# t-0hmura/pdb2reaction

Hardware: AMD Instinct MI355X
Metric: path_opt_string_iterations_per_s (higher is better)
Workload: dtype bf16x3-split

## Files before the change

### pdb2reaction_amd/csrc/umx_api.hip

```cpp
#include "umx_engine.h"
#include "umx_launch.h"
#include "umx_workspace.h"
#include "umx_periodic.h"
#include "umx_virial.h"
#include "umx_plan.h"
#include "umx_weights.h"
#include "umx_experts.h"

#define NOT_MERGED "expert-form weights are loaded but not merged: call umx_set_expert_coefficients first (then umx_set_system)"

namespace {
int energy_forces_dev_impl(umx_engine* eng, int n_images, const PosPtr d_pos, double* d_energy, float* d_forces, double* d_virial, void* hip_stream) {
  if (!eng) return UMX_ERR_ARG;
  if (eng->need_merge()) return fail(eng, UMX_ERR_ARG, "umx_energy_forces: " NOT_MERGED);
  if (!eng->have_system) return fail(eng, UMX_ERR_ARG, "umx_energy_forces: bind a system first (umx_set_system)");
  if (n_images <= 0 || !(d_pos.f || d_pos.d) || !d_energy) return fail(eng, UMX_ERR_ARG, "umx_energy_forces: bad arguments");
  if (d_virial && !d_forces) return fail(eng, UMX_ERR_ARG, "umx_energy_forces_virial: the virial comes out of the reverse pass: ask for the forces too");
  if (eng->gp_plan) return fail(eng, UMX_ERR_ARG, "umx_energy_forces: a graph-parallel evaluation is in progress (finish it with umx_gp_step)");
  CHK(periodic_check_images(eng, n_images, "umx_energy_forces"));
  HIPCHK(eng, hipSetDevice(eng->dev));
  return energy_forces_on(eng, static_cast<hipStream_t>(hip_stream), n_images, d_pos, d_energy, d_forces, d_virial);
}

template <typename P>
// ... 145 lines not shown
  if (hipGetDeviceCount(&n) != hipSuccess || n <= 0) { g_create_err = "umx_create: no HIP device visible"; return UMX_ERR_NO_DEVICE; }
  if (device_ordinal < 0 || device_ordinal >= n) { g_create_err = "umx_create: device ordinal out of range"; return UMX_ERR_ARG; }
  hipDeviceProp_t prop;
  if (hipGetDeviceProperties(&prop, device_ordinal) != hipSuccess) { g_create_err = "umx_create: hipGetDeviceProperties failed"; return UMX_ERR_HIP; }
  if (std::string(prop.gcnArchName).rfind("gfx950", 0) != 0) {
    g_create_err = std::string("umx_create: device is ") + prop.gcnArchName + ", this library is built for gfx950 only";
    return UMX_ERR_NO_DEVICE;
  }
  umx_engine* e = new umx_engine();
  e->dev = device_ordinal;
  if (const char* ev = std::getenv("UMX_STREAMS")) e->n_lanes = std::atoi(ev) >= 2 ? 2 : (std::atoi(ev) == 1 ? 1 : 0);
  if (const char* ev = std::getenv("UMX_LANES_AUTO_EDGES")) e->lanes_auto_edges = std::max(0L, std::atol(ev));
  if (const char* ev = std::getenv("UMX_FORCE_PARTS")) e->force_parts = std::max(0, std::min(16, std::atoi(ev)));
  if (const char* ev = std::getenv("UMX_RECOMPUTE")) e->recompute = std::max(0, std::min(2, std::atoi(ev)));
  if (const char* ev = std::getenv("UMX_WS_GB")) e->ws_cap_default = (size_t)std::max(0L, std::atol(ev)) << 30;
  if (const char* ev = std::getenv("UMX_WS_EAGER")) e->ws_eager = std::atoi(ev) != 0;
  if (const char* ev = std::getenv("UMX_WS_SOFT_EDGES")) e->ws_soft_edges = std::max(1L, std::atol(ev));
  if (const char* ev = std::getenv("UMX_NODE_F64")) e->node_f64_on = std::atoi(ev) != 0;
  if (const char* ev = std::getenv("UMX_GRID_F64")) e->grid_f64 = std::atoi(ev) != 0;
  if (const char* ev = std::getenv("UMX_ALT_ROWS")) e->odd_sign = std::atoi(ev) != 0 ? -1.0f : 1.0f;
  if (const char* ev = std::getenv("UMX_LOW_SEP")) e->low_sep = std::atoi(ev);
  if (const char* ev = std::getenv("UMX_GEMM_HALF")) e->gemm_half = std::atoi(ev);
  if (const char* ev = std::getenv("UMX_ALIGN_PLANES")) e->align = std::atoi(ev);
  int prio_lo = 0, prio_hi = 0;
  if (hipSetDevice(device_ordinal) != hipSuccess || hipDeviceGetStreamPriorityRange(&prio_lo, &prio_hi) != hipSuccess ||
      hipStreamCreateWithFlags(&e->stream, hipStreamNonBlocking) != hipSuccess ||
      hipStreamCreateWithPriority(&e->stream2, hipStreamNonBlocking, prio_hi) != hipSuccess ||
      hipEventCreateWithFlags(&e->ev_fork, hipEventDisableTiming) != hipSuccess || hipEventCreateWithFlags(&e->ev_join, hipEventDisableTiming) != hipSuccess ||
      hipEventCreateWithFlags(&e->ev_tok[0], hipEventDisableTiming) != hipSuccess || hipEventCreateWithFlags(&e->ev_tok[1], hipEventDisableTiming) != hipSuccess ||
      hipEventCreateWithFlags(&e->ev_done, hipEventDisableTiming) != hipSuccess || hipMalloc(&e->d_flags, 4 * sizeof(int)) != hipSuccess ||
      hipMemset(e->d_flags, 0, 4 * sizeof(int)) != hipSuccess) {
    g_create_err = "umx_create: hipSetDevice/hipStreamCreate failed";
    delete e;
    return UMX_ERR_HIP;
  }
  *out = e;
  return UMX_OK;
}


int umx_destroy(umx_engine* eng) {
  if (!eng) return UMX_OK;
  gp_clear(eng);
  (void)hipSetDevice(eng->dev);
  (void)hipStreamSynchronize(eng->stream);
  for (auto& r : eng->prof) { (void)hipEventDestroy(r.a); (void)hipEventDestroy(r.b); }
// ... 156 lines not shown
    return fail(eng, UMX_ERR_ARG, "umx_gp_begin: recompute mode 2 (umx_set_recompute / UMX_RECOMPUTE=2) is a one-GPU plan; the multi-GPU graph-parallel mode "
                                  "keeps every rank's activations stored: set mode 0 or 1 on the engines that take part");
  if (eng->pin_on)
    return fail(eng, UMX_ERR_ARG, "umx_gp_begin: a graph is pinned (umx_pin_graph) and the graph-parallel entries build their own: call umx_unpin_graph first");
  if (eng->pbc_on && eng->n_cells > 1)
    return fail(eng, UMX_ERR_ARG, "umx_gp_begin: one image, but umx_set_cells bound cells for " + std::to_string(eng->n_cells) +
                                  " images: the graph-parallel mode takes per-image cells only when exactly one is bound");
  if (eng->gp_plan) gp_clear(eng);
  HIPCHK(eng, hipSetDevice(eng->dev));
  eng->gp = true; eng->gp_lo = node_lo; eng->gp_hi = node_hi;
  const int st = energy_forces_on(eng, static_cast<hipStream_t>(hip_stream), 1, d_pos, d_energy, d_forces, d_virial);
  if (st != UMX_OK) gp_clear(eng);
  return st;
}

int umx_gp_step(umx_engine* eng, float** d_buf, size_t* count, int* done) {
  if (!eng || !d_buf || !count || !done) return UMX_ERR_ARG;
  if (!eng->gp_plan) return fail(eng, UMX_ERR_ARG, "umx_gp_step: no graph-parallel evaluation in progress (umx_gp_begin)");
  HIPCHK(eng, hipSetDevice(eng->dev));
  hipStream_t own = eng->stream;
  eng->stream = eng->gp_stream;
  *d_buf = nullptr; *count = 0; *done = 0;
  const Seg* stop = nullptr;
  int st = eng->gp_plan->run_to_sync(eng->gp_at, &stop);
  eng->stream = own;
  if (stop) { *d_buf = stop->sync_buf; *count = stop->sync_count; return UMX_OK; }
  if (st == UMX_OK) {
    *done = 1;
    eng->ran_on_caller = true;
    hipError_t e = hipEventRecord(eng->ev_done, eng->gp_stream);
    if (e != hipSuccess) st = fail(eng, UMX_ERR_HIP, std::string("umx_gp_step: ") + hipGetErrorName(e));
  }
  gp_clear(eng);
  return st;
}

namespace {
struct PeerState {
  hipEvent_t ev_in[PEER_MAX] = {}, ev_out[PEER_MAX] = {};
  int ev_dev[PEER_MAX];
  std::set<std::pair<int, int>> enabled;
  PeerState() { for (int& d : ev_dev) d = -1; }
} g_peer;

int peer_fail(int code, const std::string& msg) { g_create_err = msg; return code; }

#define PEERCHK(expr)                                                                                          \
// ... 273 lines not shown
```

### pdb2reaction_amd/csrc/umx_engine.h

```cpp
#pragma once
#include <hip/hip_runtime.h>
#include <algorithm>
#include <cmath>
#include <cstdio>
#include <cstdlib>
#include <chrono>
#include <cstring>
#include <functional>
#include <initializer_list>
#include <map>
#include <memory>
#include <set>
#include <string>
#include <type_traits>
#include <vector>

#include "../../include/umx.h"
#include "umx_common.h"
#include "umx_gemm.h"
#include "umx_gemm_pl.h"
#include "umx_gemm_q.h"
#include "umx_kernels_pl.h"
#include "umx_kernels.h"
#include "umx_radial.h"
// ... 86 lines not shown
struct WS {
  int *deg, *row_ptr, *stats;
  float* xs[2 * NL + 1];
  float* xn[NL];
  float *xn2, *ffhg, *xf, *pre1, *pre2, *enode;
  float* gspre[NL];
  float* ffh[NL];
  float* ffg1[NL];
  float* ffg2[NL];
  float *gridA, *gridB;
  float *G0, *G1, *G2, *ggs, *n128a, *n128b;
  int *esrc, *edst, *ez, *out_ptr, *out_cur, *out_edge;
  float *evec, *frame, *dedd, *dedd_rad, *tau, *tau2, *gvec;
  float* h1pre[NL + 1];
  float* h2pre[NL + 1];
  float *ra, *rad_deg;
  float* rad[NL];
  float* hg[NL];
  float* msg[NL];
  float *xrot, *hid, *gmsg, *ghg, *gy1, *grad, *e128a;
  unsigned short *y1pl, *hidpl, *a2pl, *gmsgpl, *ghgpl, *gradpl;
};

struct Seg { bool matrix; std::function<int()> fn; float* sync_buf = nullptr; size_t sync_count = 0; };
struct Plan {
  std::vector<Seg> segs;
  void stream(std::function<int()> f) { segs.push_back({false, std::move(f)}); }
  void matrix(std::function<int()> f) { segs.push_back({true, std::move(f)}); }
  void sync(float* buf, size_t count) { Seg sg{false, nullptr}; sg.sync_buf = buf; sg.sync_count = count; segs.push_back(std::move(sg)); }
  int run_to_sync(size_t& at, const Seg** stop) {
    *stop = nullptr;
    while (at < segs.size()) {
      Seg& sg = segs[at++];
      if (sg.sync_buf) { *stop = &sg; return UMX_OK; }
      const int st = sg.fn();
      if (st != UMX_OK) return st;
    }
    return UMX_OK;
  }
};

}

struct umx_engine {
  int dev = 0;
  hipStream_t stream = nullptr;
  hipEvent_t ev_done = nullptr;
  bool ran_on_caller = false;
  int* d_flags = nullptr;
  hipStream_t stream2 = nullptr;
  hipEvent_t ev_fork = nullptr, ev_join = nullptr;
  hipEvent_t ev_tok[2] = {nullptr, nullptr};
  Precision prec;
  std::string precision;
  int low_sep = 3;
  int gemm_half = 5;
  int align = 2;
  float odd_sign = -1.0f;
  bool node_ctx = false;
  bool node_f64_on = true;
  int n_lanes = 0;
  long lanes_auto_edges = 0;
  int stream_cap = 512;
  bool throttle = false;
  bool gp = false; long gp_lo = 0, gp_hi = 0;
  std::unique_ptr<Plan> gp_plan;
  std::unique_ptr<WS> gp_ws;
  size_t gp_at = 0;
  hipStream_t gp_stream = nullptr;
  std::string err;
  bool have_weights = false;
  float* d_w = nullptr;
  float* d_dw = nullptr;
  double* d_dtab = nullptr;
  unsigned short* d_bw = nullptr;
  std::map<const float*, PlaneCopy> planes;
  std::map<std::string, Tensor> wt;
  std::vector<float> h_w;
  size_t n_w = 0, n_dw = 0, n_bw = 0;
  int n_experts = 0;
  bool experts_merged = false;
  float* d_ex = nullptr;
  MergeJob* d_mjobs = nullptr; PackJob* d_pjobs = nullptr; unsigned* d_mx = nullptr;
  int n_mjobs = 0, n_pjobs = 0, merge_blocks = 0, pack_blocks = 0;
  std::vector<const float*> f16_keys;
// ... 82 lines not shown
  std::vector<ProfRec> prof;
  size_t prof_used = 0;
  bool dbg_on = false;
  std::map<std::string, std::vector<char>> dbg;
};

namespace {

#define HIPCHK(eng, expr)                                                                         \
  do {                                                                                            \
    hipError_t _e = (expr);                                                                       \
    if (_e != hipSuccess) {                                                                       \
      (eng)->err = std::string(#expr) + ": " + hipGetErrorName(_e) + " (" + hipGetErrorString(_e) + ")"; \
      return UMX_ERR_HIP;                                                                         \
    }                                                                                             \
  } while (0)

#define CHK(expr) do { int _s = (expr); if (_s != UMX_OK) return _s; } while (0)

int fail(umx_engine* e, int code, const std::string& msg) { e->err = msg; return code; }

inline unsigned nblk(long n, int per) { return (unsigned)((n + per - 1) / per); }

struct DevBuf {
  void** p; size_t bytes;
  template <class T> DevBuf(T*& ptr, size_t count) : p(reinterpret_cast<void**>(&ptr)), bytes(count * sizeof(T)) {}
};
template <class Cap>
int grow(umx_engine* eng, Cap& cap, Cap new_cap, std::initializer_list<hipStream_t> drain, std::initializer_list<DevBuf> bufs) {
  for (hipStream_t s : drain) HIPCHK(eng, hipStreamSynchronize(s));
  for (const DevBuf& b : bufs) if (*b.p) HIPCHK(eng, hipFree(*b.p));
  for (const DevBuf& b : bufs) *b.p = nullptr;
  cap = 0;
  for (const DevBuf& b : bufs) HIPCHK(eng, hipMalloc(b.p, b.bytes));
  cap = new_cap;
  return UMX_OK;
}
inline long grown_edges(long e) { return e + e / 50 + 1024; }
int grow_arena(umx_engine* eng, hipStream_t s, size_t bytes) {
  CHK(grow(eng, eng->arena_bytes, bytes, {s, eng->stream2}, {DevBuf(eng->arena, bytes)}));
  ++eng->arena_allocs;
  return UMX_OK;
}

bool dbg_wanted(const std::string& name) {
  const char* ev = std::getenv("UMX_DEBUG_ONLY");
// ... 23 lines not shown
```

### pdb2reaction_amd/csrc/umx_plan.h

```cpp
#pragma once

namespace {

enum OpFmt {
  OP_QUAD,
  OP_HALVES,
  OP_PLANES,
  OP_ROWS
};
OpFmt fwd_operand(const Precision& p) { return !p.planes ? OP_ROWS : p.fwd_fmt == 1 ? OP_HALVES : OP_QUAD; }
OpFmt rev_operand(const Precision& p) { return p.rev_quad() ? OP_QUAD : OP_PLANES; }
std::string link_tag(int slot) { return slot == NL ? ".deg" : "." + std::to_string(slot); }
int dbg_operand(umx_engine* eng, const char* base, int slot, OpFmt fmt, const void* ptr, long ne, long cols, int planes = 2) {
  if (!eng->dbg_on) return UMX_OK;
  const long rows = (fmt == OP_QUAD || fmt == OP_HALVES) ? (ne + 3) / 4 * 4 : ne;
  const size_t elem = fmt == OP_PLANES ? 2 * (size_t)planes : 4;
  return dbg_capture(eng, std::string(base) + (fmt == OP_QUAD ? "q" : fmt == OP_HALVES ? "h" : fmt == OP_PLANES ? "pl" : "") + link_tag(slot), ptr, (size_t)rows * cols * elem);
}

#define UMX_LAUNCH(kernel, grid, ...) hipLaunchKernelGGL(kernel, dim3(grid), dim3(256), 0, eng->stream, __VA_ARGS__)

int link_radial_head(umx_engine* eng, const WS& w, const RadialW& r, int slot, long ne) {
  const bool planes = eng->prec.planes && eng->planes.count(r.w3);
  const unsigned tiles = nblk(ne, 64);
// ... 73 lines not shown
  HIPCHK(eng, hipGetLastError());
  DBG("dedd_rad" + t, w.dedd_rad, ne);
  return UMX_OK;
}
int radial_bwd(umx_engine* eng, const WS& w, const RadialW& r, int slot, long ne, const float* grad, const unsigned short* gradpl = nullptr) {
  CHK(radial_bwd_fc3(eng, w, r, ne, grad, gradpl));
  return radial_bwd_tail(eng, w, r, slot, ne);
}

struct ChunkCtx {
  umx_engine* eng;
  long nn, ne, nimg;
  long img0;
  bool gp;
  long g_lo, g_hi;
  bool pinned;
  long pin_e0, pin_ecnt;
  bool may_trunc;
  bool rc;
  bool fused_rev;
  PosPtr d_pos; const int *d_deg, *d_cand;
  double* d_energy; float* d_forces;
  VirialOut vir;
};
#define UMX_STAGE(c) umx_engine* const eng = (c).eng; const hipStream_t s = eng->stream; const long nn = (c).nn, ne = (c).ne; (void)s; (void)nn; (void)ne

int graph_build(const ChunkCtx& c, const WS& w) {
  UMX_STAGE(c);
  launch_scan(s, c.d_deg, nn, w.row_ptr, w.stats);
  if (c.pinned) launch_graph_replay(eng, s, c.d_pos, c.nimg, c.pin_e0, c.pin_ecnt, w.esrc, w.edst, w.evec, c.img0);
  else launch_graph_fill(eng, s, c.may_trunc, c.d_pos, nn, c.d_cand, w.row_ptr, w.esrc, w.edst, w.evec, c.g_lo, c.g_hi, c.img0);
  HIPCHK(eng, hipMemsetAsync(w.out_cur, 0, (nn + 1) * sizeof(int), s));
  if (ne > 0) UMX_LAUNCH(k_out_count, nblk(ne, 256), w.esrc, ne, w.out_cur);
  launch_scan(s, w.out_cur, nn, w.out_ptr, w.stats + 2);
  HIPCHK(eng, hipMemsetAsync(w.out_cur, 0, (nn + 1) * sizeof(int), s));
  if (ne > 0) {
    UMX_LAUNCH(k_out_fill, nblk(ne, 256), w.esrc, ne, w.out_ptr, w.out_cur, w.out_edge);
    UMX_LAUNCH(k_out_sort, nblk(nn, 4), w.out_ptr, nn, w.out_edge);
    UMX_LAUNCH(k_edge_geom, nblk(ne, 256), w.evec, ne, eng->cutoff, w.frame);
    UMX_LAUNCH(k_edge_z, nblk(ne, 256), w.esrc, w.edst, eng->d_z, eng->natoms, w.ez, ne);
  }
  HIPCHK(eng, hipGetLastError());
  DBG("row_ptr", w.row_ptr, nn + 1); DBG("src", w.esrc, ne); DBG("dst", w.edst, ne); DBG("out_ptr", w.out_ptr, nn + 1); DBG("out_edge", w.out_edge, ne);
  DBG("evec", w.evec, ne * 4); DBG("frame", w.frame, ne * FRAME);
  return UMX_OK;
}

int edge_degree_embed(const ChunkCtx& c, const WS& w) {
  UMX_STAGE(c);
  if (ne > 0) {
    CHK(link_radial_head(eng, w, eng->rdeg, NL, ne));
    CHK(radial_fwd_fc3(eng, w, eng->rdeg, ne, w.rad_deg));
  }
  if (c.gp) UMX_LAUNCH(k_rotate_back_reduce<3>, nblk(nn, 4), w.rad_deg, w.frame, w.row_ptr, (const float*)nullptr, w.G1, nn, DEG_RESCALE,
                       (const int*)nullptr, 0, (const float*)nullptr, (const double*)nullptr);
  else UMX_LAUNCH(k_rotate_back_reduce<3>, nblk(nn, 4), w.rad_deg, w.frame, w.row_ptr, (const float*)nullptr, w.xs[0], nn, DEG_RESCALE,
                  (const int*)eng->d_z, eng->natoms, eng->emb_sphere, (const double*)eng->d_sysemb);
  HIPCHK(eng, hipGetLastError());
  if (!c.gp) { DBG("rad.deg", w.rad_deg, ne * 3 * C); DBG("x0", w.xs[0], nn * ROW); DBG("h1pre.deg", w.h1pre[NL], ne * RH); DBG("h2pre.deg", w.h2pre[NL], ne * RH); }
  return UMX_OK;
}

void plan_graph(Plan& P, WS& w, const ChunkCtx& c) {
  P.stream([c, &w]() -> int { CHK(graph_build(c, w)); return edge_degree_embed(c, w); });
  if (!c.gp) return;
  P.sync(w.G1, (size_t)c.nn * ROW);
  P.stream([c, &w]() -> int {
    UMX_STAGE(c);
    UMX_LAUNCH(k_node_init_add, nblk(nn * ROW, 256), eng->d_z, eng->natoms, nn, eng->emb_sphere, eng->d_sysemb, w.G1, w.xs[0]);
    HIPCHK(eng, hipGetLastError());
    return UMX_OK;
  });
}

void norm1_fwd(const ChunkCtx& c, const WS& w, int i) {
  UMX_STAGE(c);
  UMX_LAUNCH(k_norm_fwd, nblk(nn, 4), w.xs[2 * i], eng->lw[i].n1w, eng->lw[i].n1b, eng->d_sysemb, w.xn[i], nn);
}
void plan_edge_fwd(Plan& P, WS& w, const ChunkCtx& c, int i, bool replay) {
  const LayerW* L = &c.eng->lw[i];
  if (c.ne > 0 && c.eng->prec.planes) {
    P.stream([=, &w]() -> int {
      if (!replay) norm1_fwd(c, w, i);
      return link_radial_head(c.eng, w, L->rad, i, c.ne);
    });
    P.matrix([=, &w]() -> int { return radial_fwd_fc3(c.eng, w, L->rad, c.ne, w.rad[i]); });
    P.stream([=, &w]() -> int { return link_gather_rotate_mod(c.eng, w, i, c.ne); });
    P.matrix([=, &w]() -> int { return so2_conv(c.eng, FWD, w.y1pl, SO2_Y1, w.hg[i], SO2_HG, L->c1m0, L->c1m1, L->c1m2, L->c1m0b, c.ne, 1.0f); });
    P.stream([=, &w]() -> int { return link_gate_fwd(c.eng, w, i, c.ne); });
    P.matrix([=, &w]() -> int { return so2_conv(c.eng, FWD, w.hidpl, SO2_MSG, w.msg[i], SO2_MSG, L->c2m0, L->c2m1, L->c2m2, L->c2m0b, c.ne, 1.0f); });
    return;
  }
  P.stream([=, &w]() -> int {
    UMX_STAGE(c);
    if (!replay) norm1_fwd(c, w, i);
    if (ne > 0) {
      UMX_LAUNCH(k_gather_rotate, nblk(ne, 4), w.xn[i], w.esrc, w.edst, w.frame, w.xrot, ne);
      CHK(radial_fwd(eng, w, L->rad, i, ne, w.rad[i]));
      CHK(so2_conv(eng, FWD, w.xrot, SO2_Y1, w.hg[i], SO2_HG, L->c1m0, L->c1m1, L->c1m2, L->c1m0b, ne, 1.0f, w.rad[i]));
      UMX_LAUNCH(k_gate_edge_fwd, nblk(ne * (H / 4), 256), w.hg[i], w.hid, ne);
      CHK(so2_conv(eng, FWD, w.hid, SO2_MSG, w.msg[i], SO2_MSG, L->c2m0, L->c2m1, L->c2m2, L->c2m0b, ne, 1.0f));
    }
    HIPCHK(eng, hipGetLastError());
    return UMX_OK;
  });
}

int aggregate_fwd(const ChunkCtx& c, const WS& w, int i) {
  UMX_STAGE(c);
// ... 23 lines not shown
  if (eng->dbg_on) DBG("ffhg" + t, w.ffhg, nn * ROW);
  return UMX_OK;
}
int atomwise_fwd_grid(const ChunkCtx& c, const WS& w, int i) {
  UMX_STAGE(c);
  const LayerW& L = eng->lw[i];
  float *xmid = w.xs[2 * i + 1], *xout = w.xs[2 * i + 2];
  const std::string t = "." + std::to_string(i);
  const int G = eng->grid_G;
  const long ng = nn * G;
  UMX_LAUNCH(k_grid_expand, nblk(nn, 4), w.xn2, eng->to_grid, G, w.gridA, nn);
  if (eng->dbg_on) DBG("gridin" + t, w.gridA, ng * C);
  CHK(gemm_grid(eng, w.gridA, C, 0, L.g1w, C, L.g1b, w.ffg1[i], H, 0, ng, H, C));
  CHK(gemm_grid(eng, w.ffg1[i], H, 0, L.g2w, H, L.g2b, w.ffg2[i], H, 0, ng, H, H, A_SILU));
  CHK(gemm_grid(eng, w.ffg2[i], H, 0, L.g3w, H, L.g3b, w.gridA, C, 0, ng, C, H, A_SILU));
  UMX_LAUNCH(k_grid_contract, nblk(nn, 4), w.gridA, eng->from_grid, G, xmid, xout, nn);
  HIPCHK(eng, hipGetLastError());
  if (eng->dbg_on) DBG("gridout" + t, w.gridA, ng * C);
  DBG("xn2" + t, w.xn2, nn * ROW); DBG("ffg1" + t, w.ffg1[i], ng * H); DBG("ffg2" + t, w.ffg2[i], ng * H); DBG("x" + t, xout, nn * ROW);
  return UMX_OK;
}

void plan_layer_fwd(Plan& P, WS& w, const ChunkCtx& c, int i) {
  plan_edge_fwd(P, w, c, i, false);
  if (c.gp) {
    P.stream([c, &w, i]() -> int {
      UMX_STAGE(c);
      UMX_LAUNCH(k_rotate_back_reduce<9>, nblk(nn, 4), w.msg[i], w.frame, w.row_ptr, (const float*)nullptr, w.xn2, nn, 1.0f,
                 (const int*)nullptr, 0, (const float*)nullptr, (const double*)nullptr);
      HIPCHK(eng, hipGetLastError());
      return UMX_OK;
    });
    P.sync(w.xn2, (size_t)c.nn * ROW);
  }
  P.stream([c, &w, i]() -> int {
    UMX_STAGE(c);
    const LayerW& L = eng->lw[i];
    CHK(aggregate_fwd(c, w, i));
    UMX_LAUNCH(k_norm_fwd, nblk(nn, 4), w.xs[2 * i + 1], L.n2w, L.n2b, (const double*)nullptr, w.xn2, nn);
    return eng->ff_grid ? atomwise_fwd_grid(c, w, i) : atomwise_fwd_spectral(c, w, i);
  });
}

int readout(const ChunkCtx& c, const WS& w) {
  UMX_STAGE(c);
  UMX_LAUNCH(k_norm_fwd, nblk(nn, 4), w.xs[2 * NL], eng->normw, eng->normb, (const double*)nullptr, w.xf, nn);
  CHK(gemm_node(eng, w.xf, ROW, 0, eng->e0, C, eng->e0b, w.pre1, H, 0, nn, H, C));
// ... 47 lines not shown
  UMX_STAGE(c);
  const LayerW& L = eng->lw[i];
  const std::string t = "." + std::to_string(i);
  const int G = eng->grid_G;
  const long ng = nn * G;
  UMX_LAUNCH(k_grid_expand, nblk(nn, 4), w.G0, eng->from_grid, G, w.gridA, nn);
  if (eng->dbg_on) DBG("g_gridout" + t, w.gridA, ng * C);
  CHK(gemm_grid(eng, w.gridA, C, 0, L.g3T, C, nullptr, w.gridB, H, 0, ng, H, C));
  if (eng->dbg_on) DBG("g_gsil2" + t, w.gridB, ng * H);
  UMX_LAUNCH(k_silu_bwd, nblk(ng * H, 256), w.gridB, (long)H, w.ffg2[i], w.gridA, ng, H);
  if (eng->dbg_on) DBG("g_ffg2" + t, w.gridA, ng * H);
  CHK(gemm_grid(eng, w.gridA, H, 0, L.g2T, H, nullptr, w.gridB, H, 0, ng, H, H));
  if (eng->dbg_on) DBG("g_gsil1" + t, w.gridB, ng * H);
  UMX_LAUNCH(k_silu_bwd, nblk(ng * H, 256), w.gridB, (long)H, w.ffg1[i], w.gridA, ng, H);
  if (eng->dbg_on) DBG("g_ffg1" + t, w.gridA, ng * H);
  CHK(gemm_grid(eng, w.gridA, H, 0, L.g1T, H, nullptr, w.gridB, C, 0, ng, C, H));
  if (eng->dbg_on) DBG("g_gridin" + t, w.gridB, ng * C);
  UMX_LAUNCH(k_grid_contract, nblk(nn, 4), w.gridB, eng->to_grid, G, (const float*)nullptr, w.G1, nn);
  if (eng->dbg_on) DBG("g_xn2" + t, w.G1, nn * ROW);
  return UMX_OK;
}

void plan_atomwise_bwd(Plan& P, WS& w, const ChunkCtx& c, int i) {
  P.stream([c, &w, i]() -> int {
    UMX_STAGE(c);
    CHK(eng->ff_grid ? atomwise_bwd_grid(c, w, i) : atomwise_bwd_spectral(c, w, i));
    UMX_LAUNCH(k_norm_bwd, nblk(nn, 4), w.G1, w.xs[2 * i + 1], eng->lw[i].n2w, w.G0, w.G2, nn);
    HIPCHK(eng, hipGetLastError());
    DBG("g_xmid." + std::to_string(i), w.G2, nn * ROW);
    if (ne > 0 && eng->prec.planes) CHK(link_rotate_back_bwd(eng, w, i, ne));
    return UMX_OK;
  });
}

void plan_edge_bwd(Plan& P, WS& w, const ChunkCtx& c, int i) {
  if (c.ne <= 0) return;
  const LayerW* L = &c.eng->lw[i];
  if (c.eng->prec.planes) {
    P.matrix([=, &w]() -> int { return so2_conv(c.eng, REV, w.gmsgpl, SO2_MSG, w.hid, SO2_MSG, L->c2m0T, L->c2m1T, L->c2m2T, nullptr, c.ne, -1.0f); });
    P.stream([=, &w]() -> int {
      UMX_STAGE(c);
      DBG("g_hid." + std::to_string(i), w.hid, ne * ROW);
      return link_gate_bwd(eng, w, i, ne);
    });
    P.matrix([=, &w]() -> int { return so2_conv(c.eng, REV, w.ghgpl, SO2_HG, w.gy1, SO2_Y1, L->c1m0T, L->c1m1T, L->c1m2T, nullptr, c.ne, -1.0f); });
    P.matrix([=, &w]() -> int {
      UMX_STAGE(c);
      DBG("g_y1." + std::to_string(i), w.gy1, ne * XROT);
      return link_modrot_bwd(eng, w, i, nn, ne);
    });
    P.matrix([=, &w]() -> int { return radial_bwd_fc3(c.eng, w, L->rad, c.ne, nullptr, w.gradpl, c.eng->prec.rev_quad()); });
    P.stream([=, &w]() -> int { return radial_bwd_tail(c.eng, w, L->rad, i, c.ne); });
    return;
  }
  P.stream([=, &w]() -> int {
    UMX_STAGE(c);
    const std::string t = "." + std::to_string(i);
    UMX_LAUNCH(k_rotate_back_bwd<9>, nblk(ne, 4), w.G2, w.msg[i], w.frame, w.edst, w.gmsg, w.dedd, w.tau, ne, 1.0f);
    CHK(so2_conv(eng, REV, w.gmsg, SO2_MSG, w.hid, SO2_MSG, L->c2m0T, L->c2m1T, L->c2m2T, nullptr, ne, -1.0f));
    DBG("g_msg" + t, w.gmsg, ne * ROW); DBG("g_hid" + t, w.hid, ne * ROW);
    UMX_LAUNCH(k_gate_edge_bwd, nblk(ne * H, 256), w.hid, w.hg[i], w.ghg, ne);
    CHK(so2_conv(eng, REV, w.ghg, SO2_HG, w.gy1, SO2_Y1, L->c1m0T, L->c1m1T, L->c1m2T, nullptr, ne, -1.0f));
    DBG("g_hg" + t, w.ghg, ne * HG); DBG("g_y1" + t, w.gy1, ne * XROT);
    if (c.fused_rev) CHK(link_modrot_bwd(eng, w, i, nn, ne));
    else {
      UMX_LAUNCH(k_gather_rotate, nblk(ne, 4), w.xn[i], w.esrc, w.edst, w.frame, w.xrot, ne);
      UMX_LAUNCH(k_modulate_bwd, nblk(ne, 4), w.gy1, w.xrot, w.rad[i], w.grad, w.tau, ne);
      DBG("g_xrot" + t, w.gy1, ne * XROT); DBG("g_rad" + t, w.grad, ne * RAD);
    }
    return radial_bwd(eng, w, L->rad, i, ne, w.grad);
  });
}

void plan_norm1_bwd(Plan& P, WS& w, const ChunkCtx& c, int i) {
  const bool have_gxn = c.ne > 0 && c.fused_rev;
// ... 18 lines not shown
    return UMX_OK;
  });
}

int force_assembly(const ChunkCtx& c, const WS& w) {
  UMX_STAGE(c);
  if (ne > 0) {
    if (c.rc) {
      CHK(link_radial_head(eng, w, eng->rdeg, NL, ne));
      CHK(radial_fwd_fc3(eng, w, eng->rdeg, ne, w.rad_deg));
    }
    CHK(link_rotate_back_bwd_deg(eng, w, ne));
    CHK(radial_bwd(eng, w, eng->rdeg, NL, ne, w.gmsg, deg_rev_planes(eng) ? w.gmsgpl : nullptr));
    if (c.fused_rev) UMX_LAUNCH(k_add4, nblk(ne, 256), w.tau, w.tau2, ne);
    UMX_LAUNCH(k_force_edge, nblk(ne, 256), w.dedd, w.dedd_rad, w.tau, w.frame, w.evec, w.gvec, ne);
  }
  UMX_LAUNCH(k_force_node, nblk(nn, 4), w.gvec, w.row_ptr, w.out_ptr, w.out_edge, (float)eng->rmsd, c.d_forces, nn);
  HIPCHK(eng, hipGetLastError());
  if (c.vir.out) CHK(virial_launch(eng, w, c.vir, c.nimg, ne));
  DBG("dedd", w.dedd, ne); DBG("tau", w.tau, ne * 4); DBG("gvec", w.gvec, ne * 4);
  return UMX_OK;
}

void plan_chunk(umx_engine* eng, WS& w, const PosPtr d_pos, const int* d_deg, const int* d_cand, long img0, long nimg, long ne, double* d_energy,
                float* d_forces, Plan& P, const VirialOut vir = VirialOut()) {
  const bool gp = eng->gp, pinned = eng->pin_on;
  const long nn = nimg * eng->natoms, g_lo = gp ? eng->gp_lo : 0, g_hi = gp ? eng->gp_hi : nn;
  const long pin_e0 = pinned && gp ? eng->pin_row[g_lo] : 0, pin_ecnt = pinned ? (gp ? eng->pin_row[g_hi] - pin_e0 : eng->pin_edges) : 0;
  const ChunkCtx c{eng, nn, ne, nimg, img0, gp, g_lo, g_hi, pinned, pin_e0, pin_ecnt, eng->may_truncate, eng->rc_active && d_forces != nullptr,
                   eng->prec.planes || !eng->dbg_on, d_pos, d_deg, d_cand, d_energy, d_forces, vir};
  plan_graph(P, w, c);
  for (int i = 0; i < NL; ++i) plan_layer_fwd(P, w, c, i);
  P.stream([c, &w]() -> int {
    CHK(readout(c, w));
    return c.d_forces ? reverse_head(c, w) : UMX_OK;
  });
  if (!d_forces) return;
  for (int i = NL - 1; i >= 0; --i) {
    if (c.rc && ne > 0 && (gp || i != NL - 1)) plan_edge_fwd(P, w, c, i, true);
    plan_atomwise_bwd(P, w, c, i);
    plan_edge_bwd(P, w, c, i);
    plan_norm1_bwd(P, w, c, i);
  }
  P.stream([c, &w]() -> int { return force_assembly(c, w); });
  if (gp) P.sync(d_forces, (size_t)nn * 3);
}
#undef UMX_STAGE
#undef UMX_LAUNCH

int run_plan(umx_engine* eng, Plan& P) {
  size_t at = 0;
  const Seg* stop = nullptr;
  CHK(P.run_to_sync(at, &stop));
  return stop ? fail(eng, UMX_ERR_ARG, "run_plan: a plan with exchange points is issued step by step (umx_gp_step, eval_partitioned)") : UMX_OK;
}

int run_plans_alternating(umx_engine* eng, Plan (&P)[2], hipStream_t (&st)[2], hipEvent_t (&tok)[2]) {
  size_t at[2] = {0, 0};
  bool recorded[2] = {false, false};
  hipStream_t keep = eng->stream;
  int stt = UMX_OK;
  while (stt == UMX_OK && (at[0] < P[0].segs.size() || at[1] < P[1].segs.size())) {
    for (int l = 0; l < 2 && stt == UMX_OK; ++l) {
      eng->stream = st[l];
      while (at[l] < P[l].segs.size()) {
        Seg& sg = P[l].segs[at[l]++];
        if (sg.matrix && recorded[1 - l]) {
          hipError_t e = hipStreamWaitEvent(st[l], tok[1 - l], 0);
          if (e != hipSuccess) { stt = fail(eng, UMX_ERR_HIP, std::string("token wait: ") + hipGetErrorName(e)); break; }
        }
        stt = sg.fn();
        if (stt != UMX_OK) break;
        if (sg.matrix) {
          hipError_t e = hipEventRecord(tok[l], st[l]);
          if (e != hipSuccess) { stt = fail(eng, UMX_ERR_HIP, std::string("token record: ") + hipGetErrorName(e)); break; }
          recorded[l] = true;
// ... 127 lines not shown
  if (total > budget) return UMX_ERR_CAPACITY;
  if (eng->arena_bytes < total) CHK(grow_arena(eng, s, total));
  eng->cap_nodes = 0; eng->cap_edges = 0;
  std::vector<WS> ws(P);
  for (int p = 0; p < P; ++p) part_carve(eng->arena, off, eng->prec, eng->ws_grid(), eng->rc_active, N, cnt[p], p, ws[p]);
  std::vector<Plan> plans(P);
  double* wpart = eng->d_vir_wp;
  const bool gp_keep = eng->gp; const long lo_keep = eng->gp_lo, hi_keep = eng->gp_hi;
  for (int p = 0; p < P; ++p) {
    eng->gp = true; eng->gp_lo = lo[p]; eng->gp_hi = hi[p];
    int* deg = eng->d_part_deg + (size_t)(2 * p) * N;
    VirialOut vir;
    if (d_virial && d_forces) { vir.out = wpart + (size_t)p * 9; vir.part = eng->d_vir_part; vir.slabs = eng->vir_slabs; }
    plan_chunk(eng, ws[p], d_pos, deg, deg + N, img, 1, cnt[p], d_energy, d_forces ? eng->d_part_f + (size_t)p * N * 3 : nullptr, plans[p], vir);
  }
  eng->gp = gp_keep; eng->gp_lo = lo_keep; eng->gp_hi = hi_keep;
  std::vector<size_t> at(P, 0);
  int st = UMX_OK;
  for (;;) {
    PartPtrs pp; pp.n = P;
    size_t count = 0; int waiting = 0;
    for (int p = 0; p < P && st == UMX_OK; ++p) {
      const Seg* stop = nullptr;
      st = plans[p].run_to_sync(at[p], &stop);
      pp.p[p] = stop ? stop->sync_buf : nullptr;
      if (stop) { count = stop->sync_count; ++waiting; }
    }
    if (st != UMX_OK || waiting == 0) break;
    if (waiting != P) { st = fail(eng, UMX_ERR_ARG, "eval_partitioned: the partitions' plans disagree on their exchange points"); break; }
    const bool is_forces = d_forces && pp.p[0] == eng->d_part_f;
    hipLaunchKernelGGL(k_sum_parts, dim3((unsigned)((count + 255) / 256)), dim3(256), 0, s, pp, count, is_forces ? d_forces : (float*)nullptr);
    hipError_t e = hipGetLastError();
    if (e != hipSuccess) { st = fail(eng, UMX_ERR_HIP, std::string("k_sum_parts: ") + hipGetErrorName(e)); break; }
    if (is_forces && d_virial) {
      hipLaunchKernelGGL(k_virial_sum_parts, dim3(1), dim3(64), 0, s, wpart, P, d_virial);
      e = hipGetLastError();
      if (e != hipSuccess) { st = fail(eng, UMX_ERR_HIP, std::string("k_virial_sum_parts: ") + hipGetErrorName(e)); break; }
    }
  }
  if (st != UMX_OK) return st;
  *edges_out = 0;
  for (int p = 0; p < P; ++p) *edges_out += cnt[p];
  *maxdeg_out = cnt[P];
  return UMX_OK;
}

int eval_images_partitioned(umx_engine* eng, hipStream_t s, long K, const PosPtr d_pos, double* d_energy, float* d_forces, size_t budget, const std::string why) {
// ... 98 lines not shown
      cn = std::max(need_nodes, eng->cap_nodes); ce = std::max(grown_edges(need_edges), eng->cap_edges);
      bytes = ws_bytes(eng, cn, ce);
    }
    if (bytes > budget) { ce = std::max(need_edges, 1L); bytes = ws_bytes(eng, cn, ce); }
    if (!(eng->arena_keep && lanes * bytes <= eng->arena_bytes)) CHK(grow_arena(eng, s, lanes * bytes));
    eng->arena_keep = false;
    eng->cap_nodes = cn; eng->cap_edges = ce;
  }
  long use_nodes = eng->cap_nodes, use_edges = eng->cap_edges;
  if (lanes == 2 && eng->arena_bytes < 2 * ws_bytes(eng, use_nodes, use_edges)) {
    const long ce = grown_edges(need_edges);
    if (2 * ws_bytes(eng, need_nodes, ce) <= eng->arena_bytes) { use_nodes = need_nodes; use_edges = ce; }
    else lanes = 1;
  }
  const size_t lane_bytes = ws_bytes(eng, use_nodes, use_edges, eng->arena, &wl[0]);
  if (lanes == 2) ws_bytes(eng, use_nodes, use_edges, eng->arena + lane_bytes, &wl[1]);
  *lanes_io = lanes;
  return UMX_OK;
}

int run_chunks(umx_engine* eng, hipStream_t s, int lanes, const ImageEdges& ie, const Chunks& c, WS (&wl)[2], const PosPtr d_pos, double* d_energy, float* d_forces) {
  const int N = eng->natoms;
  int st = UMX_OK;
  auto plan_of = [&](size_t ci, int lane, Plan& P) {
    const long k0 = c.img[ci].first, k1 = c.img[ci].second;
    long e = 0;
    for (long k = k0; k < k1; ++k) e += ie.per_image[k];
    VirialOut vir;
    if (eng->vir_out && d_forces) { vir.out = eng->vir_out + k0 * 9; vir.part = eng->d_vir_part + k0 * eng->vir_slabs * 9; vir.slabs = eng->vir_slabs; }
    plan_chunk(eng, wl[lane], d_pos.atom(k0 * N), eng->pin_on ? eng->d_pin_deg : eng->d_deg_all + k0 * N, eng->pin_on ? nullptr : eng->d_cand_all + k0 * N, k0, k1 - k0, e, d_energy + k0,
               d_forces ? d_forces + k0 * N * 3 : nullptr, P, vir);
  };
  if (lanes == 2) {
    HIPCHK(eng, hipEventRecord(eng->ev_fork, s));
    HIPCHK(eng, hipStreamWaitEvent(eng->stream2, eng->ev_fork, 0));
    hipStream_t sts[2] = {s, std::getenv("UMX_LANES_ONE_STREAM") ? s : eng->stream2};
    hipEvent_t tok[2] = {eng->ev_tok[0], eng->ev_tok[1]};
    for (size_t ci = 0; ci < c.img.size() && st == UMX_OK; ci += 2) {
      Plan P[2];
      plan_of(ci, 0, P[0]);
      if (ci + 1 < c.img.size()) {
        plan_of(ci + 1, 1, P[1]);
        eng->throttle = true;
        st = run_plans_alternating(eng, P, sts, tok);
        eng->throttle = false;
      } else {
// ... 88 lines not shown
```

Before: 1.957.

## Fork independent edge-side work onto a second stream within each plan

Adds side/join segments to the Plan so that, for small graphs, independent work runs on stream2 while the main stream continues. Edge geometry and degree radial overlap with the out-list build, the next layer's radial MLP overlaps with aggregation and the atomwise step, and the backward radial fc3 and tail overlap with the node part. Each fork is joined with events before dependent work. This targets GPU idle time from serial small kernels, at the cost of extra event record/wait calls and the risk of missing dependencies or contention between the two streams.

```diff
diff --git a/pdb2reaction_amd/csrc/umx_api.hip b/pdb2reaction_amd/csrc/umx_api.hip
--- a/pdb2reaction_amd/csrc/umx_api.hip
+++ b/pdb2reaction_amd/csrc/umx_api.hip
@@ -191,6 +191,8 @@
   if (const char* ev = std::getenv("UMX_LOW_SEP")) e->low_sep = std::atoi(ev);
   if (const char* ev = std::getenv("UMX_GEMM_HALF")) e->gemm_half = std::atoi(ev);
   if (const char* ev = std::getenv("UMX_ALIGN_PLANES")) e->align = std::atoi(ev);
+  if (const char* ev = std::getenv("UMX_SIDE_NODE")) e->side_node = std::max(0, std::min(3, std::atoi(ev)));
+  if (const char* ev = std::getenv("UMX_DEBUG_FAIL_SEG")) e->dbg_fail_seg = std::max(0, std::atoi(ev));
   int prio_lo = 0, prio_hi = 0;
   if (hipSetDevice(device_ordinal) != hipSuccess || hipDeviceGetStreamPriorityRange(&prio_lo, &prio_hi) != hipSuccess ||
       hipStreamCreateWithFlags(&e->stream, hipStreamNonBlocking) != hipSuccess ||
@@ -393,7 +395,7 @@
   eng->stream = eng->gp_stream;
   *d_buf = nullptr; *count = 0; *done = 0;
   const Seg* stop = nullptr;
-  int st = eng->gp_plan->run_to_sync(eng->gp_at, &stop);
+  int st = eng->gp_plan->run_to_sync(eng, eng->gp_at, &stop);
   eng->stream = own;
   if (stop) { *d_buf = stop->sync_buf; *count = stop->sync_count; return UMX_OK; }
   if (st == UMX_OK) {
diff --git a/pdb2reaction_amd/csrc/umx_engine.h b/pdb2reaction_amd/csrc/umx_engine.h
--- a/pdb2reaction_amd/csrc/umx_engine.h
+++ b/pdb2reaction_amd/csrc/umx_engine.h
@@ -132,22 +132,23 @@
   unsigned short *y1pl, *hidpl, *a2pl, *gmsgpl, *ghgpl, *gradpl;
 };
 
-struct Seg { bool matrix; std::function<int()> fn; float* sync_buf = nullptr; size_t sync_count = 0; };
+struct Seg { bool matrix; std::function<int()> fn; float* sync_buf = nullptr; size_t sync_count = 0; bool side = false, join = false; };
 struct Plan {
   std::vector<Seg> segs;
   void stream(std::function<int()> f) { segs.push_back({false, std::move(f)}); }
   void matrix(std::function<int()> f) { segs.push_back({true, std::move(f)}); }
+  void side(std::function<int()> f) { Seg sg{false, std::move(f)}; sg.side = true; segs.push_back(std::move(sg)); }
+  void join() { Seg sg{false, nullptr}; sg.join = true; segs.push_back(std::move(sg)); }
   void sync(float* buf, size_t count) { Seg sg{false, nullptr}; sg.sync_buf = buf; sg.sync_count = count; segs.push_back(std::move(sg)); }
-  int run_to_sync(size_t& at, const Seg** stop) {
-    *stop = nullptr;
-    while (at < segs.size()) {
-      Seg& sg = segs[at++];
-      if (sg.sync_buf) { *stop = &sg; return UMX_OK; }
-      const int st = sg.fn();
-      if (st != UMX_OK) return st;
-    }
-    return UMX_OK;
-  }
+  int run_to_sync(umx_engine* eng, size_t& at, const Seg** stop);
+
+ private:
+  hipStream_t main_ = nullptr;
+  bool in_side_ = false;
+  bool pending_ = false;
+  int side_begin(umx_engine* eng);
+  int side_end(umx_engine* eng);
+  int side_join(umx_engine* eng);
 };
 
 }
@@ -171,6 +172,10 @@
   bool node_f64_on = true;
   int n_lanes = 0;
   long lanes_auto_edges = 0;
+  int side_node = -1;
+  long side_auto_edges = 131072;
+  int plan_lanes = 1;
+  int dbg_fail_seg = 0;
   int stream_cap = 512;
   bool throttle = false;
   bool gp = false; long gp_lo = 0, gp_hi = 0;
@@ -299,6 +304,53 @@
 
 inline unsigned nblk(long n, int per) { return (unsigned)((n + per - 1) / per); }
 
+int Plan::side_begin(umx_engine* eng) {
+  if (pending_) CHK(side_join(eng));
+  main_ = eng->stream;
+  HIPCHK(eng, hipEventRecord(eng->ev_fork, main_));
+  HIPCHK(eng, hipStreamWaitEvent(eng->stream2, eng->ev_fork, 0));
+  eng->stream = eng->stream2;
+  in_side_ = true;
+  return UMX_OK;
+}
+int Plan::side_end(umx_engine* eng) {
+  eng->stream = main_;
+  in_side_ = false;
+  pending_ = true;
+  HIPCHK(eng, hipEventRecord(eng->ev_join, eng->stream2));
+  return UMX_OK;
+}
+int Plan::side_join(umx_engine* eng) {
+  if (in_side_) CHK(side_end(eng));
+  if (!pending_) return UMX_OK;
+  pending_ = false;
+  HIPCHK(eng, hipStreamWaitEvent(eng->stream, eng->ev_join, 0));
+  return UMX_OK;
+}
+int Plan::run_to_sync(umx_engine* eng, size_t& at, const Seg** stop) {
+  *stop = nullptr;
+  int st = UMX_OK;
+  while (st == UMX_OK && at < segs.size()) {
+    Seg& sg = segs[at++];
+    if (in_side_ && !sg.side) st = side_end(eng);
+    if (st != UMX_OK) break;
+    if (sg.sync_buf) {
+      st = side_join(eng);
+      if (st == UMX_OK) { *stop = &sg; return UMX_OK; }
+      break;
+    }
+    if (sg.join) { st = side_join(eng); continue; }
+    if (sg.side && !in_side_) st = side_begin(eng);
+    if (st != UMX_OK) break;
+    if (eng->dbg_fail_seg > 0 && --eng->dbg_fail_seg == 0) st = fail(eng, UMX_ERR_ARG, "plan segment " + std::to_string(at - 1) + ": failed on request (debug)");
+    else st = sg.fn();
+  }
+  const std::string why = eng->err;
+  const int stj = side_join(eng);
+  if (st != UMX_OK) { eng->err = why; return st; }
+  return stj;
+}
+
 struct DevBuf {
   void** p; size_t bytes;
   template <class T> DevBuf(T*& ptr, size_t count) : p(reinterpret_cast<void**>(&ptr)), bytes(count * sizeof(T)) {}
diff --git a/pdb2reaction_amd/csrc/umx_plan.h b/pdb2reaction_amd/csrc/umx_plan.h
--- a/pdb2reaction_amd/csrc/umx_plan.h
+++ b/pdb2reaction_amd/csrc/umx_plan.h
@@ -119,14 +119,20 @@
   PosPtr d_pos; const int *d_deg, *d_cand;
   double* d_energy; float* d_forces;
   VirialOut vir;
+  int forks;
 };
 #define UMX_STAGE(c) umx_engine* const eng = (c).eng; const hipStream_t s = eng->stream; const long nn = (c).nn, ne = (c).ne; (void)s; (void)nn; (void)ne
 
-int graph_build(const ChunkCtx& c, const WS& w) {
+int graph_edges(const ChunkCtx& c, const WS& w) {
   UMX_STAGE(c);
   launch_scan(s, c.d_deg, nn, w.row_ptr, w.stats);
   if (c.pinned) launch_graph_replay(eng, s, c.d_pos, c.nimg, c.pin_e0, c.pin_ecnt, w.esrc, w.edst, w.evec, c.img0);
   else launch_graph_fill(eng, s, c.may_trunc, c.d_pos, nn, c.d_cand, w.row_ptr, w.esrc, w.edst, w.evec, c.g_lo, c.g_hi, c.img0);
+  HIPCHK(eng, hipGetLastError());
+  return UMX_OK;
+}
+int graph_out_lists(const ChunkCtx& c, const WS& w) {
+  UMX_STAGE(c);
   HIPCHK(eng, hipMemsetAsync(w.out_cur, 0, (nn + 1) * sizeof(int), s));
   if (ne > 0) UMX_LAUNCH(k_out_count, nblk(ne, 256), w.esrc, ne, w.out_cur);
   launch_scan(s, w.out_cur, nn, w.out_ptr, w.stats + 2);
@@ -134,21 +140,33 @@
   if (ne > 0) {
     UMX_LAUNCH(k_out_fill, nblk(ne, 256), w.esrc, ne, w.out_ptr, w.out_cur, w.out_edge);
     UMX_LAUNCH(k_out_sort, nblk(nn, 4), w.out_ptr, nn, w.out_edge);
+  }
+  HIPCHK(eng, hipGetLastError());
+  return UMX_OK;
+}
+int graph_edge_geom(const ChunkCtx& c, const WS& w) {
+  UMX_STAGE(c);
+  if (ne > 0) {
     UMX_LAUNCH(k_edge_geom, nblk(ne, 256), w.evec, ne, eng->cutoff, w.frame);
     UMX_LAUNCH(k_edge_z, nblk(ne, 256), w.esrc, w.edst, eng->d_z, eng->natoms, w.ez, ne);
   }
   HIPCHK(eng, hipGetLastError());
+  return UMX_OK;
+}
+int graph_captures(const ChunkCtx& c, const WS& w) {
+  UMX_STAGE(c);
   DBG("row_ptr", w.row_ptr, nn + 1); DBG("src", w.esrc, ne); DBG("dst", w.edst, ne); DBG("out_ptr", w.out_ptr, nn + 1); DBG("out_edge", w.out_edge, ne);
   DBG("evec", w.evec, ne * 4); DBG("frame", w.frame, ne * FRAME);
   return UMX_OK;
 }
 
+int edge_degree_radial(const ChunkCtx& c, const WS& w) {
+  if (c.ne <= 0) return UMX_OK;
+  CHK(link_radial_head(c.eng, w, c.eng->rdeg, NL, c.ne));
+  return radial_fwd_fc3(c.eng, w, c.eng->rdeg, c.ne, w.rad_deg);
+}
 int edge_degree_embed(const ChunkCtx& c, const WS& w) {
   UMX_STAGE(c);
-  if (ne > 0) {
-    CHK(link_radial_head(eng, w, eng->rdeg, NL, ne));
-    CHK(radial_fwd_fc3(eng, w, eng->rdeg, ne, w.rad_deg));
-  }
   if (c.gp) UMX_LAUNCH(k_rotate_back_reduce<3>, nblk(nn, 4), w.rad_deg, w.frame, w.row_ptr, (const float*)nullptr, w.G1, nn, DEG_RESCALE,
                        (const int*)nullptr, 0, (const float*)nullptr, (const double*)nullptr);
   else UMX_LAUNCH(k_rotate_back_reduce<3>, nblk(nn, 4), w.rad_deg, w.frame, w.row_ptr, (const float*)nullptr, w.xs[0], nn, DEG_RESCALE,
@@ -159,7 +177,19 @@
 }
 
 void plan_graph(Plan& P, WS& w, const ChunkCtx& c) {
-  P.stream([c, &w]() -> int { CHK(graph_build(c, w)); return edge_degree_embed(c, w); });
+  if (c.forks & 1) {
+    P.stream([c, &w]() -> int { return graph_edges(c, w); });
+    P.side([c, &w]() -> int { CHK(graph_edge_geom(c, w)); return edge_degree_radial(c, w); });
+    P.stream([c, &w]() -> int { return graph_out_lists(c, w); });
+    P.join();
+    P.stream([c, &w]() -> int { return edge_degree_embed(c, w); });
+    return;
+  }
+  P.stream([c, &w]() -> int {
+    CHK(graph_edges(c, w)); CHK(graph_out_lists(c, w)); CHK(graph_edge_geom(c, w)); CHK(graph_captures(c, w));
+    CHK(edge_degree_radial(c, w));
+    return edge_degree_embed(c, w);
+  });
   if (!c.gp) return;
   P.sync(w.G1, (size_t)c.nn * ROW);
   P.stream([c, &w]() -> int {
@@ -174,14 +204,16 @@
   UMX_STAGE(c);
   UMX_LAUNCH(k_norm_fwd, nblk(nn, 4), w.xs[2 * i], eng->lw[i].n1w, eng->lw[i].n1b, eng->d_sysemb, w.xn[i], nn);
 }
-void plan_edge_fwd(Plan& P, WS& w, const ChunkCtx& c, int i, bool replay) {
+void plan_edge_fwd(Plan& P, WS& w, const ChunkCtx& c, int i, bool replay, bool headed = false) {
   const LayerW* L = &c.eng->lw[i];
   if (c.ne > 0 && c.eng->prec.planes) {
-    P.stream([=, &w]() -> int {
-      if (!replay) norm1_fwd(c, w, i);
-      return link_radial_head(c.eng, w, L->rad, i, c.ne);
-    });
-    P.matrix([=, &w]() -> int { return radial_fwd_fc3(c.eng, w, L->rad, c.ne, w.rad[i]); });
+    if (!headed) {
+      P.stream([=, &w]() -> int {
+        if (!replay) norm1_fwd(c, w, i);
+        return link_radial_head(c.eng, w, L->rad, i, c.ne);
+      });
+      P.matrix([=, &w]() -> int { return radial_fwd_fc3(c.eng, w, L->rad, c.ne, w.rad[i]); });
+    }
     P.stream([=, &w]() -> int { return link_gather_rotate_mod(c.eng, w, i, c.ne); });
     P.matrix([=, &w]() -> int { return so2_conv(c.eng, FWD, w.y1pl, SO2_Y1, w.hg[i], SO2_HG, L->c1m0, L->c1m1, L->c1m2, L->c1m0b, c.ne, 1.0f); });
     P.stream([=, &w]() -> int { return link_gate_fwd(c.eng, w, i, c.ne); });
@@ -251,7 +283,25 @@
 }
 
 void plan_layer_fwd(Plan& P, WS& w, const ChunkCtx& c, int i) {
-  plan_edge_fwd(P, w, c, i, false);
+  const bool fork = (c.forks & 1) != 0;
+  plan_edge_fwd(P, w, c, i, false, fork && i > 0);
+  if (fork && i + 1 < NL) {
+    const LayerW* Ln = &c.eng->lw[i + 1];
+    P.stream([c, &w, i]() -> int { return aggregate_fwd(c, w, i); });
+    P.side([=, &w]() -> int { return link_radial_head(c.eng, w, Ln->rad, i + 1, c.ne); });
+    P.side([=, &w]() -> int { return radial_fwd_fc3(c.eng, w, Ln->rad, c.ne, w.rad[i + 1]); });
+    P.stream([c, &w, i]() -> int {
+      UMX_STAGE(c);
+      const LayerW& L = eng->lw[i];
+      UMX_LAUNCH(k_norm_fwd, nblk(nn, 4), w.xs[2 * i + 1], L.n2w, L.n2b, (const double*)nullptr, w.xn2, nn);
+      CHK(eng->ff_grid ? atomwise_fwd_grid(c, w, i) : atomwise_fwd_spectral(c, w, i));
+      norm1_fwd(c, w, i + 1);
+      HIPCHK(eng, hipGetLastError());
+      return UMX_OK;
+    });
+    P.join();
+    return;
+  }
   if (c.gp) {
     P.stream([c, &w, i]() -> int {
       UMX_STAGE(c);
@@ -345,13 +395,23 @@
 }
 
 void plan_atomwise_bwd(Plan& P, WS& w, const ChunkCtx& c, int i) {
-  P.stream([c, &w, i]() -> int {
+  auto node_part = [c, &w, i]() -> int {
     UMX_STAGE(c);
     CHK(eng->ff_grid ? atomwise_bwd_grid(c, w, i) : atomwise_bwd_spectral(c, w, i));
     UMX_LAUNCH(k_norm_bwd, nblk(nn, 4), w.G1, w.xs[2 * i + 1], eng->lw[i].n2w, w.G0, w.G2, nn);
     HIPCHK(eng, hipGetLastError());
     DBG("g_xmid." + std::to_string(i), w.G2, nn * ROW);
-    if (ne > 0 && eng->prec.planes) CHK(link_rotate_back_bwd(eng, w, i, ne));
+    return UMX_OK;
+  };
+  if (c.forks & 2) {
+    P.stream(node_part);
+    if (i + 1 < NL) P.join();
+    P.stream([c, &w, i]() -> int { return link_rotate_back_bwd(c.eng, w, i, c.ne); });
+    return;
+  }
+  P.stream([c, &w, i, node_part]() -> int {
+    CHK(node_part());
+    if (c.ne > 0 && c.eng->prec.planes) CHK(link_rotate_back_bwd(c.eng, w, i, c.ne));
     return UMX_OK;
   });
 }
@@ -372,8 +432,10 @@
       DBG("g_y1." + std::to_string(i), w.gy1, ne * XROT);
       return link_modrot_bwd(eng, w, i, nn, ne);
     });
-    P.matrix([=, &w]() -> int { return radial_bwd_fc3(c.eng, w, L->rad, c.ne, nullptr, w.gradpl, c.eng->prec.rev_quad()); });
-    P.stream([=, &w]() -> int { return radial_bwd_tail(c.eng, w, L->rad, i, c.ne); });
+    auto fc3T = [=, &w]() -> int { return radial_bwd_fc3(c.eng, w, L->rad, c.ne, nullptr, w.gradpl, c.eng->prec.rev_quad()); };
+    auto tail = [=, &w]() -> int { return radial_bwd_tail(c.eng, w, L->rad, i, c.ne); };
+    if (c.forks & 2) { P.side(fc3T); P.side(tail); }
+    else { P.matrix(fc3T); P.stream(tail); }
     return;
   }
   P.stream([=, &w]() -> int {
@@ -438,13 +500,19 @@
   return UMX_OK;
 }
 
+int side_forks(const umx_engine* eng, long ne) {
+  const bool plain = !eng->gp && !eng->rc_active && eng->plan_lanes == 1 && eng->prec.planes && !eng->dbg_on && ne > 0;
+  if (!plain) return 0;
+  return eng->side_node >= 0 ? eng->side_node : (ne <= eng->side_auto_edges ? 3 : 0);
+}
+
 void plan_chunk(umx_engine* eng, WS& w, const PosPtr d_pos, const int* d_deg, const int* d_cand, long img0, long nimg, long ne, double* d_energy,
                 float* d_forces, Plan& P, const VirialOut vir = VirialOut()) {
   const bool gp = eng->gp, pinned = eng->pin_on;
   const long nn = nimg * eng->natoms, g_lo = gp ? eng->gp_lo : 0, g_hi = gp ? eng->gp_hi : nn;
   const long pin_e0 = pinned && gp ? eng->pin_row[g_lo] : 0, pin_ecnt = pinned ? (gp ? eng->pin_row[g_hi] - pin_e0 : eng->pin_edges) : 0;
   const ChunkCtx c{eng, nn, ne, nimg, img0, gp, g_lo, g_hi, pinned, pin_e0, pin_ecnt, eng->may_truncate, eng->rc_active && d_forces != nullptr,
-                   eng->prec.planes || !eng->dbg_on, d_pos, d_deg, d_cand, d_energy, d_forces, vir};
+                   eng->prec.planes || !eng->dbg_on, d_pos, d_deg, d_cand, d_energy, d_forces, vir, side_forks(eng, ne)};
   plan_graph(P, w, c);
   for (int i = 0; i < NL; ++i) plan_layer_fwd(P, w, c, i);
   P.stream([c, &w]() -> int {
@@ -458,6 +526,7 @@
     plan_edge_bwd(P, w, c, i);
     plan_norm1_bwd(P, w, c, i);
   }
+  if (c.forks & 2) P.join();
   P.stream([c, &w]() -> int { return force_assembly(c, w); });
   if (gp) P.sync(d_forces, (size_t)nn * 3);
 }
@@ -467,7 +536,7 @@
 int run_plan(umx_engine* eng, Plan& P) {
   size_t at = 0;
   const Seg* stop = nullptr;
-  CHK(P.run_to_sync(at, &stop));
+  CHK(P.run_to_sync(eng, at, &stop));
   return stop ? fail(eng, UMX_ERR_ARG, "run_plan: a plan with exchange points is issued step by step (umx_gp_step, eval_partitioned)") : UMX_OK;
 }
 
@@ -641,7 +710,7 @@
     size_t count = 0; int waiting = 0;
     for (int p = 0; p < P && st == UMX_OK; ++p) {
       const Seg* stop = nullptr;
-      st = plans[p].run_to_sync(at[p], &stop);
+      st = plans[p].run_to_sync(eng, at[p], &stop);
       pp.p[p] = stop ? stop->sync_buf : nullptr;
       if (stop) { count = stop->sync_count; ++waiting; }
     }
@@ -786,6 +855,7 @@
 int run_chunks(umx_engine* eng, hipStream_t s, int lanes, const ImageEdges& ie, const Chunks& c, WS (&wl)[2], const PosPtr d_pos, double* d_energy, float* d_forces) {
   const int N = eng->natoms;
   int st = UMX_OK;
+  eng->plan_lanes = lanes;
   auto plan_of = [&](size_t ci, int lane, Plan& P) {
     const long k0 = c.img[ci].first, k1 = c.img[ci].second;
     long e = 0;
```

After: 1.960, median of 4. About the same (+0.2%).
